# eduard-permyakov/permafrost-engine

Measured on AMD Instinct MI355X. Metric: agent-steps/sec (+ flow-field cells/sec), every chunk field rebuilt + every agent stepped per tick, higher is better.
Workload: dtype u64-bitmask/u8 fields, f32 agents (f64 exp); 1 GPU; BASELINE configs[2]: 1024x1024 cells, 64 flow fields = 16384 chunk fields, 100000 agents; map_chunks=16, flow_fields=64, agents=100000, hz=20, dynamic_obstacles=0, parallelism=requests by destination + uid slabs x1, 1 all-gather (16 B/agent) per tick, ranks=1, rccl_ranks=1, backend=none, tile_exchange=auto, requests=reference planner fixture, has_dest_los=device lookup, initial_velocities=flow aligned, fields_ahead=True, tick_driver=c (navhip_tick_run), library=libnavhip.so (in-tree)

## Files before the change

permafrost-engine_amd/csrc/field_kernels.hip:

```cpp
#include "navhip_internal.h"

#include "wave_bits.h"

__device__ __forceinline__ bool req_uses_bfs(const nh_map_view &map, const navhip_field_req &rq,
                                             int force_generic)
{
    if(force_generic) return false;
    if(rq.type == NAVHIP_TARGET_NEAREST_PATHABLE || (rq.flags & NAVHIP_REQ_ISLAND_NEAREST)) return false;
    const nh_layer_view &L = map.layers[rq.layer];
    return L.unit_cost[(int)rq.chunk_r * map.w + rq.chunk_c] != 0;
}

__device__ __forceinline__ uint16_t portal_first_iid(const uint16_t *li, int r0, int c0, int r1, int c1)
{
    for(int r = r0; r <= r1; r++)
        for(int c = c0; c <= c1; c++) {
            const uint16_t v = li[r * 64 + c];
            if(v != NAVHIP_ISLAND_NONE) return v;
        }
    return NAVHIP_ISLAND_NONE;
}

__device__ __forceinline__ bool req_prepare(const nh_map_view &map, navhip_field_req &rq)
{
// ... 45 lines not shown
{
    if(rq.next_chunk_r < rq.chunk_r) return NAVHIP_FD_N;
    if(rq.next_chunk_r > rq.chunk_r) return NAVHIP_FD_S;
    if(rq.next_chunk_c < rq.chunk_c) return NAVHIP_FD_W;
    return NAVHIP_FD_E;
}

__global__ __launch_bounds__(256) void k_derive(const uint8_t *cost, const uint16_t *blockers,
                                                uint64_t *passmask, uint64_t *probemask, uint8_t *unit_cost,
                                                const uint8_t *factions, uint64_t *facmask, uint16_t *facany,
                                                const uint32_t *chunk_list, int n)
{
    int wave = (blockIdx.x * 256 + threadIdx.x) >> 6;
    int lane = threadIdx.x & 63;
    if(wave >= n) return;
    uint32_t chunk = chunk_list ? chunk_list[wave] : (uint32_t)wave;
    const uint8_t  *cb = cost + ((size_t)chunk << 12);
    const uint16_t *bl = blockers ? blockers + ((size_t)chunk << 12) : nullptr;
    uint64_t mine = 0, path = 0, blocked = 0;
    bool nonunit = false;
    for(int r = 0; r < 64; r++) {
        uint32_t cst = cb[r * 64 + lane];
        uint32_t blk = bl ? bl[r * 64 + lane] : 0;
        uint64_t m = __ballot(cst != NAVHIP_COST_IMPASSABLE && blk == 0);
        uint64_t mp = __ballot(cst != NAVHIP_COST_IMPASSABLE), mb = __ballot(blk > 0);
        nonunit |= (cst != NAVHIP_COST_IMPASSABLE && cst != 1);
        if(lane == r) { mine = m; path = mp; blocked = mb; }
    }
    passmask[(size_t)chunk * 64 + lane] = mine;
    probemask[((size_t)chunk * 64 + lane) * 2]     = path;
    probemask[((size_t)chunk * 64 + lane) * 2 + 1] = blocked;
    bool any_nonunit = __any(nonunit);
    if(lane == 0) unit_cost[chunk] = any_nonunit ? 0 : 1;
    if(factions) {
        const uint8_t *fa = factions + ((size_t)chunk * NAVHIP_MAX_FACTIONS << 12) + lane * 64;
        uint32_t any = 0;
        for(int f = 0; f < NAVHIP_MAX_FACTIONS; f++) {
            const uint64_t m = nz_row_mask(fa + ((size_t)f << 12));
            facmask[((size_t)chunk * NAVHIP_MAX_FACTIONS + f) * 64 + lane] = m;
            if(__ballot(m != 0)) any |= 1u << f;
        }
        if(lane == 0) facany[chunk] = (uint16_t)any;
    }
}

void nh_launch_derive(navhip_ctx *ctx, int layer, const uint32_t *d_chunk_list, int n, hipStream_t s)
{
    navhip_layer &L = ctx->layers[layer];
    int blocks = (n + 3) / 4;
    hipLaunchKernelGGL(k_derive, dim3(blocks), dim3(256), 0, s, L.cost, L.blockers, L.passmask, L.probemask,
                       L.unit_cost, L.factions, L.facmask, L.facany, d_chunk_list, n);
}

__device__ __forceinline__ uint64_t faction_pass_row(const nh_layer_view &L, int chunk, int lane, uint32_t enemies)
{
    const uint64_t *pm = L.probemask + ((size_t)chunk * 64 + lane) * 2;
    const uint64_t path = pm[0], blocked = pm[1];
    if(!L.facmask) return path;
    uint64_t friends = 0;
    uint32_t fs = __builtin_amdgcn_readfirstlane((int)(L.facany[chunk] & ~enemies & ((1u << NAVHIP_MAX_FACTIONS) - 1u)));
    const uint64_t *fm = L.facmask + (size_t)chunk * NAVHIP_MAX_FACTIONS * 64 + lane;
    while(fs) {
        const int f = __builtin_ctz(fs);
        fs &= fs - 1;
        friends |= fm[f * 64];
    }
    return path & ~(blocked & friends);
}

#define NH_MAXP 12
#define BFS_WAVES 4

template <bool WANT_INTEG>
__global__ __launch_bounds__(BFS_WAVES * 64) void k_field_bfs(nh_map_view map, const navhip_field_req *reqs,
                                                   int n, uint8_t *dirs, float *integ,
                                                   int force_generic, int32_t *gen_list, int gen_slot,
                                                   const int32_t *out_slot)
{
    __shared__ __attribute__((aligned(16))) uint8_t stage[BFS_WAVES][NH_CELLS];

    const int wib  = threadIdx.x >> 6;
    const int wave = blockIdx.x * BFS_WAVES + wib;
    const int lane = threadIdx.x & 63;
    if(wave >= n) return;

    navhip_field_req rq = reqs[wave];
    if(!req_uses_bfs(map, rq, force_generic)) {
        if(lane == 0) gen_list[2 + atomicAdd(&gen_list[gen_slot], 1)] = wave;
        return;
    }
    if(!req_prepare(map, rq)) return;

    const nh_layer_view &L = map.layers[rq.layer];
    const int chunk = (int)rq.chunk_r * map.w + rq.chunk_c;
    const u64x pass = mk(rq.faction_id == NAVHIP_FACTION_ID_NONE ? L.passmask[(size_t)chunk * 64 + lane]
                                                                 : faction_pass_row(L, chunk, lane, rq.enemies));

    u64x seeds = u64x{0, 0};
    if(rq.type == NAVHIP_TARGET_TILE) {
        if(lane == rq.tile_r) seeds = mk(1ull << rq.tile_c) & pass;
    }else{
        if(rq.port_c0 == rq.port_c1) {
            bool s = portal_seed(map, rq, lane, rq.port_c0, (to64(pass) >> rq.port_c0) & 1);
            if(s) seeds = mk(1ull << rq.port_c0);
        }else{
            for(int r = rq.port_r0; r <= rq.port_r1; r++) {
                uint64_t prow = __shfl(to64(pass), r);
                bool s = portal_seed(map, rq, r, lane, (prow >> lane) & 1);
                uint64_t m = __ballot(s);
                if(lane == r) seeds = mk(m);
            }
        }
    }

    u64x open = andn(pass, seeds);
    u64x frontier = seeds;
    u64x pl[NH_MAXP];
#pragma unroll
    for(int k = 0; k < NH_MAXP; k++) pl[k] = u64x{0, 0};

    int level = 0;
#define NH_BFS_LEVEL(NLOW)                                                                   \
    {                                                                                        \
        u64x nw = bfs_reach(frontier, open);                                                 \
        if(!__any(nz(nw))) break;                                                            \
        level++;                                                                             \
        pl[0] = pl[0] ^ open;                                                                \
        if(NLOW > 1) pl[1] = pl[1] ^ open;                                                   \
        if(NLOW > 2) pl[2] = pl[2] ^ open;                                                   \
        if(NLOW > 3) {                                                                       \
            const int tz = __builtin_ctz(level);          \
            _Pragma("unroll")                                                                \
            for(int k = 3; k < NH_MAXP; k++) {                                               \
                if(k <= tz) pl[k] = pl[k] ^ open;                                            \
            }                                                                                \
        }                                                                                    \
        open = andn(open, nw);                                                               \
        frontier = nw;                                                                       \
    }
    for(;;) {
        NH_BFS_LEVEL(1) NH_BFS_LEVEL(2) NH_BFS_LEVEL(1) NH_BFS_LEVEL(3)
        NH_BFS_LEVEL(1) NH_BFS_LEVEL(2) NH_BFS_LEVEL(1) NH_BFS_LEVEL(4)
    }
#undef NH_BFS_LEVEL
    const u64x reach = andn(pass, open);
#pragma unroll
    for(int k = 0; k < NH_MAXP; k++) pl[k] = pl[k] & reach;

    const int P = 32 - __builtin_clz((unsigned)level + 1);

    if(WANT_INTEG) {
        float *out = integ + ((size_t)wave << 12);
        for(int c = 0; c < 64; c++) {
            uint32_t d = 0;
#pragma unroll
            for(int k = 0; k < NH_MAXP; k++) d |= (uint32_t)((to64(pl[k]) >> c) & 1) << k;
            bool fin = (to64(reach) >> c) & 1;
            out[lane * 64 + c] = fin ? (float)d : __builtin_inff();
        }
    }

    u64x anybit = u64x{0, 0};
#pragma unroll
    for(int k = 0; k < NH_MAXP; k++) anybit = anybit | pl[k];
    const u64x zero = andn(reach, anybit);
    const u64x act  = reach & anybit;

    const u64x rN = from_n(reach), rS = from_s(reach), rW = from_w(reach), rE = from_e(reach);
    u64x eqN, eqS, eqW, eqE;
    {
        const u64x m0 = pl[0], m1 = pl[1];
        u64x n0, n1;
        n0 = from_n(pl[0]); n1 = from_n(pl[1]); eqN = andn(n0 ^ m0, n1 ^ n0 ^ m1) & rN;
        n0 = from_s(pl[0]); n1 = from_s(pl[1]); eqS = andn(n0 ^ m0, n1 ^ n0 ^ m1) & rS;
        n0 = from_w(pl[0]); n1 = from_w(pl[1]); eqW = andn(n0 ^ m0, n1 ^ n0 ^ m1) & rW;
        n0 = from_e(pl[0]); n1 = from_e(pl[1]); eqE = andn(n0 ^ m0, n1 ^ n0 ^ m1) & rE;
    }

    u64x neNW = u64x{0, 0}, neNE = neNW, neSW = neNW, neSE = neNW;
    {
        u64x b1 = u64x{~0u, ~0u};
        u64x b2 = u64x{~0u, ~0u};
#pragma unroll
        for(int k = 0; k < NH_MAXP; k++) {
            if(k < P) {
                u64x e = pl[k] ^ b1;  b1 = andn(b1, pl[k]);
                u64x f = e ^ b2;      b2 = andn(b2, e);
                u64x up = from_n(pl[k]), dn = from_s(pl[k]);
                neNW = neNW | (from_w(up) ^ f);
                neNE = neNE | (from_e(up) ^ f);
                neSW = neSW | (from_w(dn) ^ f);
                neSE = neSE | (from_e(dn) ^ f);
            }
        }
    }
    const u64x eqNW = andn(from_w(rN), neNW), eqNE = andn(from_e(rN), neNE);
    const u64x eqSW = andn(from_w(rS), neSW), eqSE = andn(from_e(rS), neSE);

    const u64x hasD = (eqNW & rN & rW) | (eqNE & rN & rE) | (eqSW & rS & rW) | (eqSE & rS & rE);
    const u64x h = act & hasD;
    const u64x g = andn(act, hasD);

    const u64x mN  = g & eqN;
    const u64x mS  = andn(g & eqS, eqN);
    const u64x mE  = andn(g & eqE, eqN | eqS);
    const u64x mW  = andn(g & eqW, eqN | eqS | eqE);
    const u64x mNW = h & eqNW;
    const u64x mNE = andn(h & eqNE, eqNW);
    const u64x mSW = andn(h & eqSW, eqNW | eqNE);
    const u64x mSE = andn(h & eqSE, eqNW | eqNE | eqSW);

    u64x D0 = mNW | mNE | mE | mS;
    u64x D1 = mN | mNE | mSW | mS;
    u64x D2 = mW | mE | mSW | mS;
    u64x D3 = mSE;
    if(rq.type == NAVHIP_TARGET_PORTAL) {
        uint32_t fd = portal_fix_dir(rq);
        if(fd & 1) D0 = D0 | zero;
        if(fd & 2) D1 = D1 | zero;
        if(fd & 4) D2 = D2 | zero;
    }

    uint8_t *out = dirs + ((size_t)(out_slot ? out_slot[wave] : wave) << 12);
    uint8_t *st = stage[wib];
    const bool inout = (rq.flags & NAVHIP_REQ_INOUT) != 0;
    if(inout) {
#pragma unroll
        for(int j = 0; j < 4; j++)
            *(uint4*)(st + j * 1024 + lane * 16) = *(const uint4*)(out + j * 1024 + lane * 16);
    }
    __builtin_amdgcn_wave_barrier();
    {
        uint32_t *row = (uint32_t*)(st + lane * 64);
        const uint64_t d0 = to64(D0), d1 = to64(D1), d2 = to64(D2), d3 = to64(D3);
        const uint64_t rc = to64(reach);
#pragma unroll
        for(int j = 0; j < 16; j++) {
            uint32_t b0 = (((uint32_t)(d0 >> (4 * j)) & 0xf) * 0x00204081u) & 0x01010101u;
            uint32_t b1 = (((uint32_t)(d1 >> (4 * j)) & 0xf) * 0x00204081u) & 0x01010101u;
            uint32_t b2 = (((uint32_t)(d2 >> (4 * j)) & 0xf) * 0x00204081u) & 0x01010101u;
            uint32_t b3 = (((uint32_t)(d3 >> (4 * j)) & 0xf) * 0x00204081u) & 0x01010101u;
            uint32_t v = b0 | (b1 << 1) | (b2 << 2) | (b3 << 3);
            if(inout) {
                uint32_t rm = ((((uint32_t)(rc >> (4 * j)) & 0xf) * 0x00204081u) & 0x01010101u) * 0xffu;
                v = (v & rm) | (row[j] & ~rm);
            }
            row[j] = v;
        }
    }
    __builtin_amdgcn_wave_barrier();
#pragma unroll
    for(int j = 0; j < 4; j++)
        *(uint4*)(out + j * 1024 + lane * 16) = *(const uint4*)(st + j * 1024 + lane * 16);
}

struct generic_lds {
    uint32_t dist[NH_CELLS];
    __attribute__((aligned(16))) uint8_t pc[NH_CELLS];
    uint8_t raw[NH_CELLS];
    uint8_t fl[NH_CELLS];
    int s_list[128], s_dmin[128], s_nlist, s_D;
};

__device__ void field_generic_one(generic_lds &S, const nh_map_view &map, const navhip_field_req *reqs,
                                  int ri, uint8_t *dirs, float *integ, int force_generic,
                                  const int32_t *out_slot)
{
    uint32_t (&dist)[NH_CELLS] = S.dist;
    uint8_t (&pc)[NH_CELLS] = S.pc;
    uint8_t (&raw)[NH_CELLS] = S.raw;
    uint8_t (&fl)[NH_CELLS] = S.fl;
    int (&s_list)[128] = S.s_list;
    int (&s_dmin)[128] = S.s_dmin;
    int &s_nlist = S.s_nlist, &s_D = S.s_D;

    const int t = threadIdx.x;
    navhip_field_req rq = reqs[ri];
    if(req_uses_bfs(map, rq, force_generic)) return;
    if(!req_prepare(map, rq)) return;

    const nh_layer_view &L = map.layers[rq.layer];
    const size_t cbase = (size_t)((int)rq.chunk_r * map.w + rq.chunk_c) << 12;
    const bool faction = rq.faction_id != NAVHIP_FACTION_ID_NONE;
    const bool modeA = rq.type == NAVHIP_TARGET_NEAREST_PATHABLE;
    const bool modeB = !modeA && (rq.flags & NAVHIP_REQ_ISLAND_NEAREST) != 0;

#pragma unroll 4
    for(int k = 0; k < 16; k++) {
        int i = k * 256 + t;
        uint32_t cst = L.cost[cbase + i];
        uint32_t blk = L.blockers ? L.blockers[cbase + i] : 0;
        bool passable;
        if(cst == NAVHIP_COST_IMPASSABLE) {
            passable = false;
        }else if(!faction) {
            passable = (blk == 0);
        }else{
            bool enemies_only = true;
            if(L.factions) {
                const uint8_t *fp = L.factions + cbase * NAVHIP_MAX_FACTIONS + i;
                for(int f = 0; f < NAVHIP_MAX_FACTIONS; f++) {
                    if(fp[(size_t)f << 12] && !(rq.enemies & (1u << f))) { enemies_only = false; break; }
                }
            }
            passable = enemies_only || (blk == 0);
        }
        pc[i] = passable ? (uint8_t)cst : (uint8_t)NAVHIP_COST_IMPASSABLE;
        raw[i] = (uint8_t)cst;
        fl[i] = (cst != NAVHIP_COST_IMPASSABLE && blk == 0) ? 1 : 0;
        dist[i] = NH_INF_U32;
    }
    if(t == 0) { s_nlist = 0; s_D = 0x7fffffff; }
    if(t < 128) s_dmin[t] = 0x7fffffff;
    __syncthreads();

    if(modeA) {
        const int start = rq.tile_r * 64 + rq.tile_c;
        if(t == 0) fl[start] |= 2;
        __syncthreads();
        if(!(fl[start] & 1)) {
            for(;;) {
                int changed = 0;
#pragma unroll 4
                for(int k = 0; k < 16; k++) {
                    int i = k * 256 + t;
                    if(fl[i] & 3) continue;
                    int r = i >> 6, c = i & 63;
                    bool nb = (r > 0 && (fl[i - 64] & 2)) || (r < 63 && (fl[i + 64] & 2))
                           || (c > 0 && (fl[i - 1] & 2)) || (c < 63 && (fl[i + 1] & 2));
// ... 116 lines not shown
                if(c < 63) m = min(m, dist[i + 1]);
                if(m < NH_INF_U32) {
                    uint32_t nd = m + cst;
                    if(nd < dist[i]) { dist[i] = nd; changed = 1; }
                }
            }
            if(!__syncthreads_or(changed)) break;
        }
    }

    const bool inout = (rq.flags & NAVHIP_REQ_INOUT) != 0 || modeA || modeB;
    uint8_t *out = dirs + ((size_t)(out_slot ? out_slot[ri] : ri) << 12);
    const uint32_t fixdir = (rq.type == NAVHIP_TARGET_PORTAL) ? portal_fix_dir(rq) : NAVHIP_FD_NONE;
    uint8_t res[16];
#pragma unroll 4
    for(int k = 0; k < 16; k++) {
        int i = k * 256 + t;
        int r = i >> 6, c = i & 63;
        uint32_t d = dist[i];
        uint32_t dir;
        if(d >= NH_INF_U32) {
            dir = inout ? out[i] : NAVHIP_FD_NONE;
        }else if(d == 0) {
            dir = modeA ? out[i] : fixdir;
        }else{
            const uint32_t I = NH_INF_U32;
            uint32_t dn = r > 0  ? dist[i - 64] : I, ds = r < 63 ? dist[i + 64] : I;
            uint32_t dw = c > 0  ? dist[i - 1]  : I, de = c < 63 ? dist[i + 1]  : I;
            uint32_t dnw = (r > 0  && c > 0)  ? dist[i - 65] : I;
            uint32_t dne = (r > 0  && c < 63) ? dist[i - 63] : I;
            uint32_t dsw = (r < 63 && c > 0)  ? dist[i + 63] : I;
            uint32_t dse = (r < 63 && c < 63) ? dist[i + 65] : I;
            uint32_t mc = min(min(dn, ds), min(dw, de));
            if(dn < I && dw < I) mc = min(mc, dnw);
            if(dn < I && de < I) mc = min(mc, dne);
            if(ds < I && dw < I) mc = min(mc, dsw);
            if(ds < I && de < I) mc = min(mc, dse);
            if(dn == mc)       dir = NAVHIP_FD_N;
            else if(ds == mc)  dir = NAVHIP_FD_S;
            else if(de == mc)  dir = NAVHIP_FD_E;
            else if(dw == mc)  dir = NAVHIP_FD_W;
            else if(dnw == mc) dir = NAVHIP_FD_NW;
            else if(dne == mc) dir = NAVHIP_FD_NE;
            else if(dsw == mc) dir = NAVHIP_FD_SW;
            else               dir = NAVHIP_FD_SE;
        }
        res[k] = (uint8_t)dir;
        if(integ) integ[((size_t)ri << 12) + i] = (d >= NH_INF_U32) ? __builtin_inff() : (float)d;
    }
    __syncthreads();
#pragma unroll
    for(int k = 0; k < 16; k++) pc[k * 256 + t] = res[k];
    __syncthreads();
    *(uint4*)(out + t * 16) = *(const uint4*)(pc + t * 16);
}

__global__ __launch_bounds__(256) void k_field_generic(nh_map_view map, const navhip_field_req *reqs,
                                                       int n, uint8_t *dirs, float *integ,
                                                       int force_generic, int32_t *gen_list, int gen_slot,
                                                       const int32_t *out_slot)
{
    __shared__ generic_lds S;
    const int count = gen_list ? gen_list[gen_slot] : n;
    if(gen_list && blockIdx.x == 0 && threadIdx.x == 0) gen_list[gen_slot ^ 1] = 0;
    for(int w = blockIdx.x; w < count; w += gridDim.x) {
        const int ri = gen_list ? gen_list[2 + w] : w;
        field_generic_one(S, map, reqs, ri, dirs, integ, force_generic, out_slot);
        __syncthreads();
    }
}

int nh_launch_fields(navhip_ctx *ctx, const navhip_field_req *d_reqs, int n, uint8_t *d_dirs,
                     float *d_integ, int32_t *d_gen_list, hipStream_t s, const int32_t *d_out_slot)
{
    nh_map_view mv;
    nh_fill_map_view(ctx, &mv);
    const int force_generic = ctx->field_kernel_mode == 1;
    const int gen_slot = force_generic ? 0 : (int)(ctx->gen_launches++ & 1);
    if(!force_generic) {
        dim3 grid((n + BFS_WAVES - 1) / BFS_WAVES);
        if(d_integ)
            hipLaunchKernelGGL(k_field_bfs<true>, grid, dim3(BFS_WAVES * 64), 0, s, mv, d_reqs, n, d_dirs,
                               d_integ, force_generic, d_gen_list, gen_slot, d_out_slot);
        else
            hipLaunchKernelGGL(k_field_bfs<false>, grid, dim3(BFS_WAVES * 64), 0, s, mv, d_reqs, n, d_dirs,
                               d_integ, force_generic, d_gen_list, gen_slot, d_out_slot);
    }
    bool heavy = force_generic;
    for(int l = 0; l < NAVHIP_NAV_LAYER_MAX; l++) heavy = heavy || (ctx->layers[l].cost && ctx->layers[l].nonunit_costs);
    const int gmax = heavy ? 2048 : 512;
    hipLaunchKernelGGL(k_field_generic, dim3(n < gmax ? n : gmax), dim3(256), 0, s, mv, d_reqs, n, d_dirs,
                       d_integ, force_generic, force_generic ? (int32_t*)nullptr : d_gen_list, gen_slot, d_out_slot);
    return force_generic ? -1 : gen_slot;
}
```

permafrost-engine_amd/csrc/navhip_api.hip:

```cpp
#include "navhip_internal.h"
#include <cmath>

#include <cstdio>
#include <cstdlib>
#include <cstring>
#include <iterator>
#include <new>
#include <vector>

struct plane_row { size_t off; size_t cell_bytes; bool dirties, zeroed; };
static const plane_row plane_rows[] = {
    {offsetof(navhip_layer, cost),          1,                   true,  false},
    {offsetof(navhip_layer, blockers),      2,                   true,  true},
    {offsetof(navhip_layer, local_islands), 2,                   false, true},
    {offsetof(navhip_layer, factions),      NAVHIP_MAX_FACTIONS, true,  true},
    {offsetof(navhip_layer, islands),       2,                   false, true},
};
static_assert(std::size(plane_rows) == NAVHIP_PLANE_COUNT && NAVHIP_PLANE_COST_BASE == 0 && NAVHIP_PLANE_BLOCKERS == 1
           && NAVHIP_PLANE_LOCAL_ISLANDS == 2 && NAVHIP_PLANE_FACTIONS == 3 && NAVHIP_PLANE_ISLANDS == 4,
              "plane_rows: one row per NAVHIP_PLANE_*, indexed by it");
struct derived_row { size_t off; size_t chunk_bytes; bool with_factions, zeroed; };
static const derived_row derived_rows[] = {
    {offsetof(navhip_layer, passmask),    64 * sizeof(uint64_t),                       false, false},
    {offsetof(navhip_layer, probemask),   128 * sizeof(uint64_t),                      false, false},
// ... 83 lines not shown

static int layer_array(navhip_ctx *ctx, void *&p, size_t bytes, bool zeroed)
{
    if(p) return NAVHIP_OK;
    HIPCHK(ctx, hipMalloc(&p, bytes));
    if(zeroed) HIPCHK(ctx, hipMemsetAsync(p, 0, bytes, ctx->stream));
    return NAVHIP_OK;
}

static int layer_prepare(navhip_ctx *ctx, int layer, int plane)
{
    navhip_layer &L = ctx->layers[layer];
    if(!L.dirty && !(L.dirty = (uint8_t*)calloc(ctx->nchunks, 1))) return NAVHIP_ERR_NOMEM;
    int rc = layer_array(ctx, plane_slot(L, plane), plane_bytes(ctx, plane), plane_rows[plane].zeroed);
    for(const derived_row &d : derived_rows)
        if(!rc && (!d.with_factions || L.factions))
            rc = layer_array(ctx, nh_member(&L, d.off), (size_t)ctx->nchunks * d.chunk_bytes, d.zeroed);
    return rc;
}

static int upload_chunks(navhip_ctx *ctx, int layer, int plane, int chunk0, int n, bool whole, const void *host, size_t bytes,
                         const char *who)
{
    const size_t per = NH_CELLS * plane_rows[plane].cell_bytes;
    if(bytes != (size_t)n * per) {
        ctx->last_error = std::string(who) + ": size mismatch";
        return NAVHIP_ERR_INVALID;
    }
    HIPCHK(ctx, hipSetDevice(ctx->device));
    int rc = layer_prepare(ctx, layer, plane);
    if(rc) return rc;
    navhip_layer &L = ctx->layers[layer];
    HIPCHK(ctx, hipMemcpyAsync((char*)plane_slot(L, plane) + (size_t)chunk0 * per, host, bytes, hipMemcpyHostToDevice, ctx->stream));
    HIPCHK(ctx, hipStreamSynchronize(ctx->stream));
    if(plane_rows[plane].dirties) {
        memset(L.dirty + chunk0, 1, n);
        L.any_dirty = true;
    }
    if(plane == NAVHIP_PLANE_COST_BASE) {
        const uint8_t *c = (const uint8_t*)host;
        bool other = false;
        for(size_t i = 0; i < bytes && !other; i++) other = c[i] != 1 && c[i] != NAVHIP_COST_IMPASSABLE;
        L.nonunit_costs = other || (!whole && L.nonunit_costs);
    }
    return NAVHIP_OK;
}

static int build_fields_on(navhip_ctx *ctx, const navhip_field_req *dev_reqs, int n, uint8_t *dev_inout_dirs,
                           float *dev_out_integ, const int32_t *dev_slots, hipStream_t s)
{
    int rc = nh_refresh_derived(ctx, s);
    if(rc) return rc;
    const void *old_list = ctx->gen_list.p;
    rc = nh_ensure_buf(ctx, ctx->gen_list, ((size_t)n + 2) * sizeof(int32_t));
    if(rc) return rc;
    if(ctx->gen_list.p != old_list) HIPCHK(ctx, hipMemsetAsync(ctx->gen_list.p, 0, 2 * sizeof(int32_t), s));
    ctx->last_fields.gen_slot = nh_launch_fields(ctx, dev_reqs, n, dev_inout_dirs, dev_out_integ, (int32_t*)ctx->gen_list.p,
                                                 s, dev_slots);
    ctx->last_fields.n = n; ctx->last_fields.stream = s;
    HIPCHK(ctx, hipGetLastError());
    ctx->counters.field_calls++; ctx->counters.chunk_fields += (uint64_t)n;
    return NAVHIP_OK;
}

int navhip_build_fields_slots_dev(navhip_ctx *ctx, const navhip_field_req *dev_reqs, int n, uint8_t *dev_fields,
                                  const int32_t *dev_slots, hipStream_t s)
{
    if(n == 0) return NAVHIP_OK;
    return build_fields_on(ctx, dev_reqs, n, dev_fields, nullptr, dev_slots, s);
}

extern "C" {

int navhip_ctx_create(navhip_ctx **out, int chunk_w, int chunk_h, int device)
{
    if(!out || chunk_w < 1 || chunk_h < 1 || chunk_w > 64 || chunk_h > 64)
        return NAVHIP_ERR_INVALID;
    *out = nullptr;
    int ndev = 0;
    if(hipGetDeviceCount(&ndev) != hipSuccess || ndev < 1 || device < 0 || device >= ndev) {
        fprintf(stderr, "navhip: no usable HIP device (count=%d, asked for %d); this library has "
                        "no CPU fallback\n", ndev, device);
        return NAVHIP_ERR_DEVICE;
    }
    navhip_ctx *ctx = new (std::nothrow) navhip_ctx();
    if(!ctx) return NAVHIP_ERR_NOMEM;
    ctx->device = device;
    ctx->w = chunk_w; ctx->h = chunk_h; ctx->nchunks = chunk_w * chunk_h;
    if(hipSetDevice(device) != hipSuccess
    || hipStreamCreateWithFlags(&ctx->stream, hipStreamNonBlocking) != hipSuccess) {
        delete ctx;
        return NAVHIP_ERR_DEVICE;
    }
    *out = ctx;
    return NAVHIP_OK;
}

void navhip_ctx_destroy(navhip_ctx *ctx)
{
    if(!ctx) return;
    hipSetDevice(ctx->device);
    hipStreamSynchronize(ctx->stream);
    navhip_comm_destroy(ctx);
    if(ctx->step.lists_pinned) hipHostFree(ctx->step.lists_pinned);
    navhip_pool_destroy(ctx);
    nh_async_destroy(ctx);
    for(navhip_layer &L : ctx->layers) {
        for(const plane_row &p : plane_rows) hipFree(nh_member(&L, p.off));
        for(const derived_row &d : derived_rows) hipFree(nh_member(&L, d.off));
        free(L.dirty);
    }
// ... 307 lines not shown
    if(!ctx || n < 0 || (n > 0 && (!dev_reqs || !dev_inout_dirs))) return NAVHIP_ERR_INVALID;
    if(n == 0) return NAVHIP_OK;
    HIPCHK(ctx, hipSetDevice(ctx->device));
    return build_fields_on(ctx, dev_reqs, n, dev_inout_dirs, dev_out_integ, nullptr,
                           stream ? (hipStream_t)stream : ctx->stream);
}

int navhip_build_fields(navhip_ctx *ctx, const navhip_field_req *reqs, int n,
                        uint8_t *inout_dirs, float *out_integ)
{
    if(!ctx || n < 0 || (n > 0 && (!reqs || !inout_dirs))) return NAVHIP_ERR_INVALID;
    if(n == 0) return NAVHIP_OK;
    HIPCHK(ctx, hipSetDevice(ctx->device));
    int rc = nh_validate_field_reqs(ctx, reqs, n);
    if(rc) return rc;
    hipStream_t s = ctx->stream;
    bool any_inout = false;
    for(int i = 0; i < n; i++)
        any_inout |= (reqs[i].flags & (NAVHIP_REQ_INOUT | NAVHIP_REQ_IF_CHANGED | NAVHIP_REQ_ISLAND_NEAREST)) != 0
                  || reqs[i].type == NAVHIP_TARGET_NEAREST_PATHABLE;
    const size_t dirs_bytes = (size_t)n * NH_CELLS, integ_bytes = dirs_bytes * sizeof(float);
    const navhip_field_req *d_reqs;
    uint8_t *d_dirs = nullptr;
    float *d_integ = nullptr;
    rc = nh_stage_in(ctx, NH_STAGE_CALL0, reqs, (size_t)n * sizeof(navhip_field_req), (const void**)&d_reqs, s);
    if(!rc) rc = any_inout ? nh_stage_in(ctx, NH_STAGE_CALL1, inout_dirs, dirs_bytes, (const void**)&d_dirs, s)
                           : nh_stage_reserve(ctx, NH_STAGE_CALL1, dirs_bytes, (void**)&d_dirs);
    if(!rc && out_integ) rc = nh_stage_reserve(ctx, NH_STAGE_CALL2, integ_bytes, (void**)&d_integ);
    if(!rc) rc = navhip_build_fields_dev(ctx, d_reqs, n, d_dirs, d_integ, s);
    if(rc) return rc;
    HIPCHK(ctx, hipMemcpyAsync(inout_dirs, d_dirs, dirs_bytes, hipMemcpyDeviceToHost, s));
    if(out_integ) HIPCHK(ctx, hipMemcpyAsync(out_integ, d_integ, integ_bytes, hipMemcpyDeviceToHost, s));
    HIPCHK(ctx, hipStreamSynchronize(s));
    return NAVHIP_OK;
}

int navhip_set_field_kernel(navhip_ctx *ctx, int mode)
{
    if(!ctx || mode < 0 || mode > 1) return NAVHIP_ERR_INVALID;
    ctx->field_kernel_mode = mode;
    return NAVHIP_OK;
}

int navhip_last_fields_split(navhip_ctx *ctx, int32_t out[2])
{
    if(!ctx || !out) return NAVHIP_ERR_INVALID;
    if(ctx->last_fields.n < 0) {
        ctx->last_error = "navhip_last_fields_split: no chunk-field build yet";
        return NAVHIP_ERR_INVALID;
    }
    HIPCHK(ctx, hipSetDevice(ctx->device));
    int32_t generic = ctx->last_fields.n;
    if(ctx->last_fields.gen_slot >= 0)
        HIPCHK(ctx, hipMemcpyAsync(&generic, (const int32_t*)ctx->gen_list.p + ctx->last_fields.gen_slot, sizeof(int32_t),
                                   hipMemcpyDeviceToHost, ctx->last_fields.stream));
    HIPCHK(ctx, hipStreamSynchronize(ctx->last_fields.stream));
    out[0] = ctx->last_fields.n - generic; out[1] = generic;
    return NAVHIP_OK;
}

uint64_t navhip_flow_field_id(const navhip_field_req *r)
{
    if(r->type == NAVHIP_TARGET_PORTAL) {
        return (((uint64_t)r->layer)            << 60)
             | (((uint64_t)r->type)             << 56)
             | (((uint64_t)(r->next_iid & 0xf)) << 48)
             | (((uint64_t)(r->port_iid & 0xf)) << 40)
             | (((uint64_t)r->port_r0)          << 34)
             | (((uint64_t)r->port_c0)          << 28)
             | (((uint64_t)r->port_r1)          << 22)
             | (((uint64_t)r->port_c1)          << 16)
             | (((uint64_t)r->chunk_r)          <<  8)
             | (((uint64_t)r->chunk_c)          <<  0);
    }
    return (((uint64_t)r->layer)   << 60)
         | (((uint64_t)r->type)    << 56)
         | (((uint64_t)r->tile_r)  << 24)
         | (((uint64_t)r->tile_c)  << 16)
         | (((uint64_t)r->chunk_r) <<  8)
         | (((uint64_t)r->chunk_c) <<  0);
}

uint64_t navhip_region_field_id(int kind, int layer, int chunk_r, int chunk_c, uint32_t a, int b, int c)
{
    const uint64_t head = (((uint64_t)layer) << 60) | (((uint64_t)kind) << 56);
    const uint64_t tail = (((uint64_t)chunk_r) << 8) | ((uint64_t)chunk_c);
    if(kind == NAVHIP_FFID_ENEMIES || kind == NAVHIP_FFID_ENTITY)
        return head | (((uint64_t)a) << 24) | tail;
    if(kind == NAVHIP_FFID_ZONE) {
        const uint32_t cen_chunk_r = a / 64u, cen_tile_r = a % 64u;
        const uint32_t cen_chunk_c = (uint32_t)b / 64u, cen_tile_c = (uint32_t)b % 64u;
        return head | (((uint64_t)(c & 0xff)) << 44) | (((uint64_t)(cen_tile_c & 0x3f)) << 38)
             | (((uint64_t)(cen_tile_r & 0x3f)) << 32) | (((uint64_t)(cen_chunk_c & 0xff)) << 24)
             | (((uint64_t)(cen_chunk_r & 0xff)) << 16) | tail;
    }
    return 0;
}

}
```

permafrost-engine_amd/csrc/navhip_internal.h:

```cpp
#pragma once
#include <hip/hip_runtime.h>
#include <stdint.h>
#include <string>
#include <vector>
#include <initializer_list>
#include <stddef.h>
#include "navhip.h"
#include "map_view.h"

static_assert(sizeof(navhip_field_req) == 32, "navhip_field_req must stay 32 bytes");
static_assert(sizeof(navhip_los_req) == 16, "navhip_los_req must stay 16 bytes");

#define NH_CELLS   4096
#define NH_RES     64
#define NH_INF_U32 0x3fffffffu

#define HIPCHK(ctx, expr)                                                                   \
    do {                                                                                    \
        hipError_t _e = (expr);                                                             \
        if(_e != hipSuccess) {                                                              \
            (ctx)->last_error = std::string(#expr) + ": " + hipGetErrorString(_e);          \
            return NAVHIP_ERR_DEVICE;                                                       \
        }                                                                                   \
    } while(0)
// ... 124 lines not shown
    NH_SB_REC_A, NH_SB_REC_V,
    NH_SB_POOL_OF,
    NH_SB_SEP, NH_SB_CNT, NH_SB_REC,
    NH_SB_MIDREC,
    NH_SB_WL_COUNT, NH_SB_WL_IDS,
    NH_SB_COH,
    NH_SB_COH_PLAN,
    NH_SB_COUNT
};

struct nh_prefetch_key {
    const float *pos_xz, *vel_xz, *radius, *arrival_sink_xz; const uint32_t *flags;
    const uint8_t *state, *arrival_flags; const int32_t *flock_members, *flock_offsets;
    int n_ents, n_flocks, hz, work_begin, work_end;
    int32_t origin_x, origin_y; int grid_w, grid_h;
};

struct nh_step_state {
    nh_buf       buf[NH_SB_COUNT];
    unsigned     scratch_moves = 0;
    unsigned     sp_builds = 0;
    int          wl_parity = 0;
    int32_t     *lists_pinned = nullptr;
    hipStream_t  aux[2] = {nullptr, nullptr};
    hipStream_t  aux_main = nullptr;
    hipEvent_t   ev_regroup = nullptr;
    bool         serial_step = false;
    struct { bool valid = false; nh_prefetch_key key = {}; } pre;
    bool         snapshot_held = false;
    hipStream_t  front_stream = nullptr;
    bool         join0_signalled = false;
    int          start_flag = NH_HO_START;
    int32_t      start_seq = 0;
    bool         regroup_pending = false;
    bool         lists_signalled = false;
    bool         step_end_signalled = false;
    hipStream_t  step_end_on = nullptr;
    int          coh_flocks = -1, coh_members = -1, coh_parity = 0;
    unsigned     coh_unique = 0;
    int64_t      coh_regroup_key[4] = {-1, -1, -1, -1}; int coh_regroup_age = 0;
    bool         profiling = false;
    hipEvent_t   ev[6] = {};
    bool         ev_valid = false;
};

struct navhip_ctx {
    int          device = 0;
    int          w = 0, h = 0, nchunks = 0;
    hipStream_t  stream = nullptr;
    navhip_layer layers[NAVHIP_NAV_LAYER_MAX];
    int          field_kernel_mode = 0;
    nh_buf       d_dirty_list;
    nh_buf       gen_list;
    unsigned     gen_launches = 0;
    struct { int n = -1, gen_slot = -1; hipStream_t stream = nullptr; } last_fields;
    nh_buf       stage[NH_STAGE_COUNT];
    navhip_counters counters = {};
    nh_buf       state_arrived, state_arrived_n;
    nh_buf       dest_query_scratch;
    nh_step_state step;
    std::string  last_error;
    struct nh_handover *ho = nullptr;
    struct nh_pool  *pool = nullptr;
    struct nh_async *async = nullptr;
    struct nh_comm  *comm = nullptr;
};

static inline void nh_fill_map_view(const navhip_ctx *ctx, nh_map_view *mv)
{
    mv->w = ctx->w; mv->h = ctx->h;
    for(int l = 0; l < NAVHIP_NAV_LAYER_MAX; l++) {
        const navhip_layer &L = ctx->layers[l];
        mv->layers[l] = nh_layer_view{L.cost, L.blockers, L.local_islands, L.factions,
                                      L.passmask, L.unit_cost, L.changed, L.islands, L.probemask,
                                      L.facmask, L.facany, L.fac_changed};
    }
}

template<class F> static inline void nh_ctx_each_buf(navhip_ctx *ctx, F f)
{
    nh_buf *one[] = {&ctx->d_dirty_list, &ctx->gen_list, &ctx->state_arrived, &ctx->state_arrived_n, &ctx->dest_query_scratch};
    for(nh_buf *b : one) f(*b);
    for(auto &b : ctx->step.buf) f(b);
    for(auto &b : ctx->stage) f(b);
}

enum { NH_STREAM_SIDE0 = 0,
       NH_STREAM_SIDE1,
       NH_STREAM_MAIN,
       NH_STREAM_FIELDS,
       NH_STREAM_COMM,
       NH_STREAM_FIXED };
int         nh_streams_for(navhip_ctx *ctx, hipStream_t main, hipStream_t out[NH_STREAM_FIXED]);
hipStream_t nh_stream_partial_for(navhip_ctx *ctx, hipStream_t main, int cu_begin, int cu_count);
bool        nh_streams_alive(int device);
void        nh_streams_forget(int device, hipStream_t s);
int         nh_ensure_side_streams(navhip_ctx *ctx, hipStream_t main);

struct nh_signal { int32_t *flag; int32_t seq; };
struct nh_handover {
    int32_t *flags;
    int32_t *status;
    int32_t *status_dev;
    int32_t  seq[NH_HO_FLAGS];
    bool       forced_events, never_events, by_events;
    hipEvent_t ev[NH_HO_FLAGS];
};
void     nh_handover_mode(navhip_ctx *ctx, bool jam);
int      nh_handover_ensure(navhip_ctx *ctx);
void     nh_handover_destroy(navhip_ctx *ctx);
nh_signal nh_handover_by_kernel(navhip_ctx *ctx, int flag, hipStream_t producer);
void     nh_handover_signal(navhip_ctx *ctx, int flag, hipStream_t producer);
void     nh_handover_wait(navhip_ctx *ctx, int flag, hipStream_t consumer, int before = -1, int after = -1);
void     nh_handover_wait2(navhip_ctx *ctx, int flag_a, int flag_b, hipStream_t consumer);
int32_t  nh_handover_seq(navhip_ctx *ctx, int flag);
void     nh_handover_wait_for(navhip_ctx *ctx, int flag, int32_t want, hipStream_t consumer);
bool     nh_handover_failed(navhip_ctx *ctx);

extern "C" int nh_validate_field_reqs(navhip_ctx *ctx, const navhip_field_req *reqs, int n);
int  navhip_build_fields_slots_dev(navhip_ctx *ctx, const navhip_field_req *dev_reqs, int n, uint8_t *dev_fields,
                                   const int32_t *dev_slots, hipStream_t s);
int  nh_ensure(navhip_ctx *ctx, nh_buf &b, size_t need);
int  nh_ensure_buf(navhip_ctx *ctx, nh_buf &b, size_t need);
int  nh_stage_reserve(navhip_ctx *ctx, nh_stage_slot slot, size_t bytes, void **dev);
int  nh_stage_in(navhip_ctx *ctx, nh_stage_slot slot, const void *host, size_t bytes, const void **dst, hipStream_t s);
int  nh_stage_world(navhip_ctx *ctx, const navhip_world *w, navhip_world *d, hipStream_t s, std::initializer_list<size_t> only = {});
void nh_async_destroy(navhip_ctx *ctx);
void nh_async_invalidate_static(navhip_ctx *ctx);
bool nh_async_resident(navhip_ctx *ctx, navhip_world *w, navhip_step_out *o);
int  nh_async_slabs(navhip_ctx *ctx, size_t in_bytes, size_t out_bytes, char **h_in, char **h_out);
bool nh_is_pinned(const void *p);
int  nh_refresh_derived(navhip_ctx *ctx, hipStream_t s);
int  nh_spatial_query_dev(navhip_ctx *ctx, const navhip_world *dev_w, const float *d_query, int nq, float range, int maxout,
                          int32_t *d_counts, uint32_t *d_ids, hipStream_t s);
const uint8_t *nh_pool_fields(const navhip_ctx *ctx);
const int32_t *nh_pool_map(const navhip_ctx *ctx);
int nh_pool_dests(const navhip_ctx *ctx);
int nh_pool_slots(const navhip_ctx *ctx);

void nh_launch_derive(navhip_ctx *ctx, int layer, const uint32_t *d_chunk_list, int n,
                      hipStream_t s);
int  nh_launch_fields(navhip_ctx *ctx, const navhip_field_req *d_reqs, int n, uint8_t *d_dirs,
                      float *d_integ, int32_t *d_gen_list, hipStream_t s,
                      const int32_t *d_out_slot = nullptr);

void nh_launch_blockers_circles(navhip_ctx *ctx, const navhip_circle *d_circles, int n, float map_x,
                                float map_z, hipStream_t s);
void nh_launch_local_islands(navhip_ctx *ctx, int layer, hipStream_t s);
void nh_launch_region_fields(navhip_ctx *ctx, const navhip_region_req *d_reqs, int n, int max_dim,
                             const int16_t *d_seeds, const int16_t *d_overlay, uint8_t *d_out,
                             size_t out_stride, hipStream_t s);
void nh_launch_los(navhip_ctx *ctx, const navhip_los_req *d_reqs, int n, const uint8_t *d_prev,
                   uint8_t *d_out, uint8_t *d_overlay, float map_x, float map_z, hipStream_t s);

enum { NH_LCS_STALE = 0, NH_LCS_REBUILT, NH_LCS_REDONE, NH_LCS_COUNT };
struct nh_los_chain_view {
    const navhip_los_req *reqs;
    const int32_t  *prev_slot;
    const uint32_t *cell;
    const uint16_t *fmask;
    const int32_t  *level_begin;
    uint8_t        *pool;
    uint8_t        *stale;
    uint8_t        *overflow;
    int32_t        *list;
    int32_t        *count;
    int32_t        *stats;
    int             slots, levels;
    float           map_x, map_z;
};
void nh_launch_los_chain_level(navhip_ctx *ctx, const nh_los_chain_view &c, int slot0, int n, hipStream_t s);
void nh_launch_los_chain_mark(navhip_ctx *ctx, const nh_los_chain_view &c, bool downstream, hipStream_t s);
void nh_launch_los_chain_stale(navhip_ctx *ctx, const nh_los_chain_view &c, int level, int slot0, int n, hipStream_t s);
```

Measured before the change: 39.29 million agent-steps/s.

## Deduplicate identical field requests via GPU hash table and broadcast leader results

Adds a pre-pass kernel that hashes each field request into a device hash table, elects one leader per set of identical requests, and links the duplicates to it. The BFS and generic field kernels skip non-leaders and copy the leader's direction and integration tiles to every member's output slot. The aim is to avoid recomputing identical chunk fields, at the cost of an extra kernel launch, atomics, double-buffered table clearing, and the serial copy chain per leader.

```diff
diff --git a/permafrost-engine_amd/csrc/field_kernels.hip b/permafrost-engine_amd/csrc/field_kernels.hip
--- a/permafrost-engine_amd/csrc/field_kernels.hip
+++ b/permafrost-engine_amd/csrc/field_kernels.hip
@@ -121,6 +121,69 @@
                        L.unit_cost, L.factions, L.facmask, L.facany, d_chunk_list, n);
 }
 
+struct __attribute__((aligned(8))) nh_class_link { int32_t next, slot; };
+struct nh_class_view {
+    int32_t *table; uint32_t tmask;
+    uint32_t tagmask;
+    int32_t *head;
+    int32_t *leader_of;
+    struct nh_class_link *link;
+    int32_t *other_table, *other_head;
+    int clear_table, clear_heads;
+};
+
+__device__ __forceinline__ bool req_reads_own_slot(const navhip_field_req &rq)
+{
+    return (rq.flags & (NAVHIP_REQ_INOUT | NAVHIP_REQ_ISLAND_NEAREST)) != 0 || rq.type == NAVHIP_TARGET_NEAREST_PATHABLE;
+}
+
+__device__ __forceinline__ uint32_t req_hash(const uint4 &a, const uint4 &b)
+{
+    uint32_t h = 0x9e3779b9u;
+    const uint32_t w[8] = {a.x, a.y, a.z, a.w, b.x, b.y, b.z, b.w};
+#pragma unroll
+    for(int k = 0; k < 8; k++) { h = (h ^ w[k]) * 0x85ebca6bu; h ^= h >> 15; }
+    h *= 0xc2b2ae35u;
+    return h ^ (h >> 16);
+}
+
+__global__ __launch_bounds__(256) void k_field_classes(nh_map_view map, const navhip_field_req *reqs, int n,
+                                                       nh_class_view cv, const int32_t *out_slot, int32_t *gen_reqs)
+{
+    const int i = blockIdx.x * 256 + threadIdx.x;
+    bool generic = false;
+    if(i < n) {
+        const uint4 a = ((const uint4*)(reqs + i))[0], b = ((const uint4*)(reqs + i))[1];
+        navhip_field_req rq;
+        __builtin_memcpy(&rq, &a, 16);
+        __builtin_memcpy((char*)&rq + 16, &b, 16);
+        generic = !req_uses_bfs(map, rq, 0);
+        int leader = i;
+        if(!req_reads_own_slot(rq)) {
+            const uint32_t h = req_hash(a, b), tag = h & cv.tagmask;
+            for(uint32_t e = h & cv.tmask;; e = (e + 1) & cv.tmask) {
+                const uint32_t got = (uint32_t)atomicCAS(&cv.table[e], 0, (int32_t)(tag | (uint32_t)(i + 1)));
+                if(got == 0) break;
+                if((got & cv.tagmask) != tag) continue;
+                const int32_t was = (int32_t)(got & ~cv.tagmask);
+                const uint4 *o = (const uint4*)(reqs + (was - 1));
+                const uint4 oa = o[0], ob = o[1];
+                if(oa.x == a.x && oa.y == a.y && oa.z == a.z && oa.w == a.w
+                && ob.x == b.x && ob.y == b.y && ob.z == b.z && ob.w == b.w) {
+                    leader = was - 1;
+                    cv.link[i] = nh_class_link{atomicExch(&cv.head[leader], i + 1), out_slot ? out_slot[i] : i};
+                    break;
+                }
+            }
+        }
+        cv.leader_of[i] = leader;
+    }
+    if(gen_reqs) {
+        const uint64_t m = __ballot(generic);
+        if(m && (threadIdx.x & 63) == 0) atomicAdd(gen_reqs, __popcll(m));
+    }
+}
+
 __device__ __forceinline__ uint64_t faction_pass_row(const nh_layer_view &L, int chunk, int lane, uint32_t enemies)
 {
     const uint64_t *pm = L.probemask + ((size_t)chunk * 64 + lane) * 2;
@@ -144,7 +207,7 @@
 __global__ __launch_bounds__(BFS_WAVES * 64) void k_field_bfs(nh_map_view map, const navhip_field_req *reqs,
                                                    int n, uint8_t *dirs, float *integ,
                                                    int force_generic, int32_t *gen_list, int gen_slot,
-                                                   const int32_t *out_slot)
+                                                   const int32_t *out_slot, nh_class_view cv)
 {
     __shared__ __attribute__((aligned(16))) uint8_t stage[BFS_WAVES][NH_CELLS];
 
@@ -152,10 +215,10 @@
     const int wave = blockIdx.x * BFS_WAVES + wib;
     const int lane = threadIdx.x & 63;
     if(wave >= n) return;
-
     navhip_field_req rq = reqs[wave];
+    if(cv.leader_of[wave] != wave) return;
     if(!req_uses_bfs(map, rq, force_generic)) {
-        if(lane == 0) gen_list[2 + atomicAdd(&gen_list[gen_slot], 1)] = wave;
+        if(lane == 0) gen_list[NH_GEN_HEADER + atomicAdd(&gen_list[gen_slot], 1)] = wave;
         return;
     }
     if(!req_prepare(map, rq)) return;
@@ -228,6 +291,9 @@
             out[lane * 64 + c] = fin ? (float)d : __builtin_inff();
         }
     }
+    int32_t member = cv.head[wave];
+    nh_class_link node = nh_class_link{0, 0};
+    if(member) node = cv.link[member - 1];
 
     u64x anybit = u64x{0, 0};
 #pragma unroll
@@ -318,9 +384,26 @@
         }
     }
     __builtin_amdgcn_wave_barrier();
-#pragma unroll
-    for(int j = 0; j < 4; j++)
-        *(uint4*)(out + j * 1024 + lane * 16) = *(const uint4*)(st + j * 1024 + lane * 16);
+    uint4 tile[4];
+#pragma unroll
+    for(int j = 0; j < 4; j++) tile[j] = *(const uint4*)(st + j * 1024 + lane * 16);
+#pragma unroll
+    for(int j = 0; j < 4; j++) *(uint4*)(out + j * 1024 + lane * 16) = tile[j];
+    while(member) {
+        uint8_t *o = dirs + ((size_t)node.slot << 12);
+        member = node.next;
+        if(member) node = cv.link[member - 1];
+#pragma unroll
+        for(int j = 0; j < 4; j++) *(uint4*)(o + j * 1024 + lane * 16) = tile[j];
+    }
+    if(WANT_INTEG) {
+        const uint4 *src = (const uint4*)(integ + ((size_t)wave << 12) + lane * 64);
+        for(int32_t m = cv.head[wave]; m; m = cv.link[m - 1].next) {
+            uint4 *dst = (uint4*)(integ + ((size_t)(m - 1) << 12) + lane * 64);
+#pragma unroll 4
+            for(int j = 0; j < 16; j++) dst[j] = src[j];
+        }
+    }
 }
 
 struct generic_lds {
@@ -333,7 +416,7 @@
 
 __device__ void field_generic_one(generic_lds &S, const nh_map_view &map, const navhip_field_req *reqs,
                                   int ri, uint8_t *dirs, float *integ, int force_generic,
-                                  const int32_t *out_slot)
+                                  const int32_t *out_slot, const nh_class_view &cv)
 {
     uint32_t (&dist)[NH_CELLS] = S.dist;
     uint8_t (&pc)[NH_CELLS] = S.pc;
@@ -344,6 +427,7 @@
     int &s_nlist = S.s_nlist, &s_D = S.s_D;
 
     const int t = threadIdx.x;
+    if(cv.leader_of[ri] != ri) return;
     navhip_field_req rq = reqs[ri];
     if(req_uses_bfs(map, rq, force_generic)) return;
     if(!req_prepare(map, rq)) return;
@@ -566,44 +650,89 @@
 #pragma unroll
     for(int k = 0; k < 16; k++) pc[k * 256 + t] = res[k];
     __syncthreads();
-    *(uint4*)(out + t * 16) = *(const uint4*)(pc + t * 16);
+    const uint4 tile = *(const uint4*)(pc + t * 16);
+    *(uint4*)(out + t * 16) = tile;
+    int32_t member = cv.head[ri];
+    nh_class_link node = member ? cv.link[member - 1] : nh_class_link{0, 0};
+    while(member) {
+        const int m = member - 1;
+        uint8_t *o = dirs + ((size_t)node.slot << 12);
+        member = node.next;
+        if(member) node = cv.link[member - 1];
+        *(uint4*)(o + t * 16) = tile;
+        if(integ) {
+#pragma unroll 4
+            for(int k = 0; k < 16; k++) {
+                const int i = k * 256 + t;
+                const uint32_t d = dist[i];
+                integ[((size_t)m << 12) + i] = (d >= NH_INF_U32) ? __builtin_inff() : (float)d;
+            }
+        }
+    }
 }
 
 __global__ __launch_bounds__(256) void k_field_generic(nh_map_view map, const navhip_field_req *reqs,
                                                        int n, uint8_t *dirs, float *integ,
                                                        int force_generic, int32_t *gen_list, int gen_slot,
-                                                       const int32_t *out_slot)
+                                                       const int32_t *out_slot, nh_class_view cv)
 {
     __shared__ generic_lds S;
     const int count = gen_list ? gen_list[gen_slot] : n;
-    if(gen_list && blockIdx.x == 0 && threadIdx.x == 0) gen_list[gen_slot ^ 1] = 0;
+    if(gen_list && blockIdx.x == 0 && threadIdx.x == 0) gen_list[gen_slot ^ 1] = gen_list[2 + (gen_slot ^ 1)] = 0;
+    for(int i = blockIdx.x * 256 + threadIdx.x; i < cv.clear_table; i += gridDim.x * 256) cv.other_table[i] = 0;
+    for(int i = blockIdx.x * 256 + threadIdx.x; i < cv.clear_heads; i += gridDim.x * 256) cv.other_head[i] = 0;
     for(int w = blockIdx.x; w < count; w += gridDim.x) {
-        const int ri = gen_list ? gen_list[2 + w] : w;
-        field_generic_one(S, map, reqs, ri, dirs, integ, force_generic, out_slot);
+        const int ri = gen_list ? gen_list[NH_GEN_HEADER + w] : w;
+        field_generic_one(S, map, reqs, ri, dirs, integ, force_generic, out_slot, cv);
         __syncthreads();
     }
 }
 
+static size_t classes_tcap(int cap)
+{
+    size_t t = 64;
+    while(t < 8 * (size_t)cap) t <<= 1;
+    return t;
+}
+size_t nh_field_classes_bytes(int cap) { return (2 * classes_tcap(cap) + 5 * (size_t)cap) * sizeof(int32_t); }
+
 int nh_launch_fields(navhip_ctx *ctx, const navhip_field_req *d_reqs, int n, uint8_t *d_dirs,
-                     float *d_integ, int32_t *d_gen_list, hipStream_t s, const int32_t *d_out_slot)
+                     float *d_integ, int32_t *d_gen_list, int32_t *d_classes, hipStream_t s, const int32_t *d_out_slot)
 {
     nh_map_view mv;
     nh_fill_map_view(ctx, &mv);
     const int force_generic = ctx->field_kernel_mode == 1;
     const int gen_slot = force_generic ? 0 : (int)(ctx->gen_launches++ & 1);
+    const int cap = ctx->classes.cap;
+    const size_t tcap = classes_tcap(cap), set = tcap + (size_t)cap;
+    const int mine = (int)(ctx->classes.builds++ & 1);
+    const size_t tsize = classes_tcap(n);
+    nh_class_view cv;
+    cv.table = d_classes + mine * set; cv.tmask = (uint32_t)(tsize - 1);
+    cv.head = cv.table + tcap;
+    const int idx_bits = 32 - __builtin_clz((unsigned)n);
+    cv.tagmask = idx_bits >= 32 ? 0u : ~((1u << idx_bits) - 1u);
+    cv.other_table = d_classes + (mine ^ 1) * set;
+    cv.other_head = cv.other_table + tcap;
+    cv.clear_table = ctx->classes.last_table; cv.clear_heads = ctx->classes.last_heads;
+    ctx->classes.last_table = (int)tsize; ctx->classes.last_heads = n;
+    cv.leader_of = d_classes + 2 * set;
+    cv.link = (nh_class_link*)(cv.leader_of + cap);
+    hipLaunchKernelGGL(k_field_classes, dim3((n + 255) / 256), dim3(256), 0, s, mv, d_reqs, n, cv, d_out_slot,
+                       force_generic ? (int32_t*)nullptr : d_gen_list + 2 + gen_slot);
     if(!force_generic) {
         dim3 grid((n + BFS_WAVES - 1) / BFS_WAVES);
         if(d_integ)
             hipLaunchKernelGGL(k_field_bfs<true>, grid, dim3(BFS_WAVES * 64), 0, s, mv, d_reqs, n, d_dirs,
-                               d_integ, force_generic, d_gen_list, gen_slot, d_out_slot);
+                               d_integ, force_generic, d_gen_list, gen_slot, d_out_slot, cv);
         else
             hipLaunchKernelGGL(k_field_bfs<false>, grid, dim3(BFS_WAVES * 64), 0, s, mv, d_reqs, n, d_dirs,
-                               d_integ, force_generic, d_gen_list, gen_slot, d_out_slot);
+                               d_integ, force_generic, d_gen_list, gen_slot, d_out_slot, cv);
     }
     bool heavy = force_generic;
     for(int l = 0; l < NAVHIP_NAV_LAYER_MAX; l++) heavy = heavy || (ctx->layers[l].cost && ctx->layers[l].nonunit_costs);
     const int gmax = heavy ? 2048 : 512;
     hipLaunchKernelGGL(k_field_generic, dim3(n < gmax ? n : gmax), dim3(256), 0, s, mv, d_reqs, n, d_dirs,
-                       d_integ, force_generic, force_generic ? (int32_t*)nullptr : d_gen_list, gen_slot, d_out_slot);
+                       d_integ, force_generic, force_generic ? (int32_t*)nullptr : d_gen_list, gen_slot, d_out_slot, cv);
     return force_generic ? -1 : gen_slot;
 }
diff --git a/permafrost-engine_amd/csrc/navhip_api.hip b/permafrost-engine_amd/csrc/navhip_api.hip
--- a/permafrost-engine_amd/csrc/navhip_api.hip
+++ b/permafrost-engine_amd/csrc/navhip_api.hip
@@ -159,11 +159,19 @@
     int rc = nh_refresh_derived(ctx, s);
     if(rc) return rc;
     const void *old_list = ctx->gen_list.p;
-    rc = nh_ensure_buf(ctx, ctx->gen_list, ((size_t)n + 2) * sizeof(int32_t));
-    if(rc) return rc;
-    if(ctx->gen_list.p != old_list) HIPCHK(ctx, hipMemsetAsync(ctx->gen_list.p, 0, 2 * sizeof(int32_t), s));
+    rc = nh_ensure_buf(ctx, ctx->gen_list, ((size_t)n + NH_GEN_HEADER) * sizeof(int32_t));
+    if(rc) return rc;
+    if(ctx->gen_list.p != old_list) HIPCHK(ctx, hipMemsetAsync(ctx->gen_list.p, 0, NH_GEN_HEADER * sizeof(int32_t), s));
+    if(n > ctx->classes.cap) {
+        const int cap = (n + n / 2 + 1) & ~1;
+        ctx->classes = {};
+        rc = nh_ensure_buf(ctx, ctx->field_classes, nh_field_classes_bytes(cap));
+        if(rc) return rc;
+        HIPCHK(ctx, hipMemsetAsync(ctx->field_classes.p, 0, nh_field_classes_bytes(cap), s));
+        ctx->classes.cap = cap;
+    }
     ctx->last_fields.gen_slot = nh_launch_fields(ctx, dev_reqs, n, dev_inout_dirs, dev_out_integ, (int32_t*)ctx->gen_list.p,
-                                                 s, dev_slots);
+                                                 (int32_t*)ctx->field_classes.p, s, dev_slots);
     ctx->last_fields.n = n; ctx->last_fields.stream = s;
     HIPCHK(ctx, hipGetLastError());
     ctx->counters.field_calls++; ctx->counters.chunk_fields += (uint64_t)n;
@@ -577,7 +585,7 @@
     HIPCHK(ctx, hipSetDevice(ctx->device));
     int32_t generic = ctx->last_fields.n;
     if(ctx->last_fields.gen_slot >= 0)
-        HIPCHK(ctx, hipMemcpyAsync(&generic, (const int32_t*)ctx->gen_list.p + ctx->last_fields.gen_slot, sizeof(int32_t),
+        HIPCHK(ctx, hipMemcpyAsync(&generic, (const int32_t*)ctx->gen_list.p + 2 + ctx->last_fields.gen_slot, sizeof(int32_t),
                                    hipMemcpyDeviceToHost, ctx->last_fields.stream));
     HIPCHK(ctx, hipStreamSynchronize(ctx->last_fields.stream));
     out[0] = ctx->last_fields.n - generic; out[1] = generic;
diff --git a/permafrost-engine_amd/csrc/navhip_internal.h b/permafrost-engine_amd/csrc/navhip_internal.h
--- a/permafrost-engine_amd/csrc/navhip_internal.h
+++ b/permafrost-engine_amd/csrc/navhip_internal.h
@@ -200,6 +200,8 @@
     int          field_kernel_mode = 0;
     nh_buf       d_dirty_list;
     nh_buf       gen_list;
+    nh_buf       field_classes;
+    struct { int cap = 0; unsigned builds = 0; int last_table = 0, last_heads = 0; } classes;
     unsigned     gen_launches = 0;
     struct { int n = -1, gen_slot = -1; hipStream_t stream = nullptr; } last_fields;
     nh_buf       stage[NH_STAGE_COUNT];
@@ -227,7 +229,7 @@
 
 template<class F> static inline void nh_ctx_each_buf(navhip_ctx *ctx, F f)
 {
-    nh_buf *one[] = {&ctx->d_dirty_list, &ctx->gen_list, &ctx->state_arrived, &ctx->state_arrived_n, &ctx->dest_query_scratch};
+    nh_buf *one[] = {&ctx->d_dirty_list, &ctx->gen_list, &ctx->field_classes, &ctx->state_arrived, &ctx->state_arrived_n, &ctx->dest_query_scratch};
     for(nh_buf *b : one) f(*b);
     for(auto &b : ctx->step.buf) f(b);
     for(auto &b : ctx->stage) f(b);
@@ -288,8 +290,10 @@
 
 void nh_launch_derive(navhip_ctx *ctx, int layer, const uint32_t *d_chunk_list, int n,
                       hipStream_t s);
+#define NH_GEN_HEADER 4
+size_t nh_field_classes_bytes(int cap);
 int  nh_launch_fields(navhip_ctx *ctx, const navhip_field_req *d_reqs, int n, uint8_t *d_dirs,
-                      float *d_integ, int32_t *d_gen_list, hipStream_t s,
+                      float *d_integ, int32_t *d_gen_list, int32_t *d_classes, hipStream_t s,
                       const int32_t *d_out_slot = nullptr);
 
 void nh_launch_blockers_circles(navhip_ctx *ctx, const navhip_circle *d_circles, int n, float map_x,
```

New measurement: 40.12 million agent-steps/s, median of 6. +2.1%, better.
